# PaulTFLi/Machine-Learning-Replications

Hardware: AMD Instinct MI355X
Metric: train_rows_per_sec (higher is better)
Workload: dtype fp32

## Files before the change

machine-learning-replications_amd/ops/csrc/svm_ws.hip:

```cpp
#include <type_traits>

#include "common.h"

namespace hfens {

struct WsProb {
  long long zoff;
  long long aoff;
  int l;
  int npos;
  double Cp, Cn;
  float ngl2e;
  int pad;
};

struct WsState {
  int done;
  int outer;
  long long inner;
  double gap;
  int nc;
  int nws;
  int nprev;
  int pad;
// ... 86 lines not shown
  }
  *total = tot;
  return base;
}

__device__ __forceinline__ void hist_add(int* hist, bool on, int bin) {
  const unsigned long long act = __ballot(on);
  if (!act) return;
  const int first = __builtin_amdgcn_readlane(bin, __builtin_ctzll(act));
  const unsigned long long same = __ballot(on && bin == first);
  if (same == act) {
    if ((threadIdx.x & 63) == __builtin_ctzll(act)) atomicAdd(&hist[first], __popcll(act));
  } else if (on) {
    atomicAdd(&hist[bin], 1);
  }
}

struct WsAux {
  unsigned* keys;
  long long n;
  unsigned long long* gkey;
};

__device__ __forceinline__ unsigned ws_key(double v) { return f32_okey((float)v); }

__device__ __forceinline__ void ws_publish_keys(const WsProb& P, int b, int t, bool valid, double a, double g,
                                                const WsAux& X) {
  double su = -kWsInf, sl = -kWsInf;
  if (valid) {
    unsigned ku = 0u, kl = 0u;
    const bool pos = t < P.npos;
    const double C = pos ? P.Cp : P.Cn;
    const double yg = pos ? g : -g;
    if (pos ? a < C : a > 0) { su = -yg; ku = ws_key(su); }
    if (pos ? a > 0 : a < C) { sl = yg; kl = ws_key(sl); }
    X.keys[P.aoff + t] = ku;
    X.keys[X.n + P.aoff + t] = kl;
  }
  su = wave_max_f64_exact(su);
  sl = wave_max_f64_exact(sl);
  if ((threadIdx.x & 63) == 0) {
    if (su > -kWsInf) atomicMax(&X.gkey[2 * b], f64_okey(su));
    if (sl > -kWsInf) atomicMax(&X.gkey[2 * b + 1], f64_okey(sl));
  }
}

__global__ __launch_bounds__(256) void ws_init_kernel(const WsProb* __restrict__ probs, const float* __restrict__ zcat,
                                                      int F, float* __restrict__ zn, double* __restrict__ alpha,
                                                      double* __restrict__ G, WsState* __restrict__ states,
                                                      WsAux X) {
  const int b = blockIdx.y;
  const WsProb P = probs[b];
  const int t = blockIdx.x * blockDim.x + threadIdx.x;
  if (blockIdx.x * blockDim.x >= P.l) return;
  if (blockIdx.x == 0 && threadIdx.x == 0) states[b] = WsState{0, 0, 0, 0.0, 0, 0, 0, 0, 0, 0, 0, 0, 0, 0};
  const bool valid = t < P.l;
  if (valid) {
    const float* z = zcat + (P.zoff + t) * F;
    float s = 0.f;
    for (int k = 0; k < F; ++k) s = fmaf(z[k], z[k], s);
    zn[P.aoff + t] = s;
    alpha[P.aoff + t] = 0.0;
    G[P.aoff + t] = -1.0;
  }
  ws_publish_keys(P, b, t, valid, 0.0, -1.0, X);
}

constexpr size_t ws_sel_lds_bytes(int Q) { return 32 * 4 + 4096 * 4 + 1024 * 4 + (size_t)Q * 4; }

template <int M, typename Emit>
__device__ __forceinline__ int ws_pick_lists(const unsigned (&ku)[M], const unsigned (&kl)[M], int t0, int k_up,
                                             int k_low, int* shi, int* binfo, int* hist, Emit emit) {
  const int tid = threadIdx.x;
  for (int i = tid; i < 4096; i += kWsThreads) hist[i] = 0;
  if (tid < 8) binfo[tid] = 0;
  __syncthreads();
#pragma unroll
  for (int m = 0; m < M; ++m) {
    hist_add(hist, ku[m] != 0u, (int)(ku[m] >> 21));
    hist_add(hist, kl[m] != 0u, 2048 + (int)(kl[m] >> 21));
  }
  __syncthreads();
  ws_find_bin(hist, k_up, k_low, shi, binfo);
  __syncthreads();
  const unsigned bu1 = binfo[0], bl1 = binfo[2];
  const int au1 = binfo[1], al1 = binfo[3];
  for (int i = tid; i < 4096; i += kWsThreads) hist[i] = 0;
  __syncthreads();
#pragma unroll
  for (int m = 0; m < M; ++m) {
    hist_add(hist, ku[m] != 0u && (ku[m] >> 21) == bu1, (int)((ku[m] >> 10) & 2047));
    hist_add(hist, kl[m] != 0u && (kl[m] >> 21) == bl1, 2048 + (int)((kl[m] >> 10) & 2047));
  }
  __syncthreads();
  ws_find_bin(hist, k_up - au1, k_low - al1, shi, binfo + 4);
  __syncthreads();
  const unsigned Tu = (bu1 << 11) | (unsigned)binfo[4], Tl = (bl1 << 11) | (unsigned)binfo[6];
  const int need_u = k_up - au1 - binfo[5], need_l = k_low - al1 - binfo[7];
  unsigned selm = 0u;
  int base = 0;
#pragma unroll
  for (int side = 0; side < 2; ++side) {
    const unsigned T = side ? Tl : Tu;
    const int need = side ? need_l : need_u;
    int wt = 0;
#pragma unroll
    for (int m = 0; m < M; ++m) {
      const unsigned k = side ? kl[m] : ku[m];
      wt += __popcll(__ballot(k && (k >> 10) == T && !((selm >> m) & 1u)));
    }
    int ttot;
    int trank = wave_base(wt, shi, &ttot);
    unsigned pick = 0u;
    int ws_cnt = 0;
#pragma unroll
    for (int m = 0; m < M; ++m) {
      const unsigned k = side ? kl[m] : ku[m];
      const bool cand = k && !((selm >> m) & 1u);
      const bool tie = cand && (k >> 10) == T;
      const unsigned long long tb = __ballot(tie);
      const bool take = cand && ((k >> 10) > T || (tie && trank + __popcll(tb & lanes_below()) < need));
      trank += __popcll(tb);
      if (take) pick |= 1u << m;
      ws_cnt += __popcll(__ballot(take));
    }
    int stot;
    int pos = base + wave_base(ws_cnt, shi, &stot);
#pragma unroll
    for (int m = 0; m < M; ++m) {
      const bool take = (pick >> m) & 1u;
      const unsigned long long tb = __ballot(take);
      if (take) emit(pos + __popcll(tb & lanes_below()), t0 + 64 * m);
      pos += __popcll(tb);
    }
    selm |= pick;
    base += stot;
  }
  return base;
}

struct WsCand {
  int* idx;
  unsigned* ku;
  unsigned* kl;
  int ncand;
};
constexpr int kWsCandM = 8;
constexpr int kWsCandBlk = kWsCandM * kWsThreads;

template <int M, int Q, bool kWriteIdx, bool kCand = false>
__device__ __forceinline__ int ws_select_body(const WsProb& P, int b, WsState* S, int* __restrict__ wsidx,
                                              int* __restrict__ wsprev, double eps, int max_outer, const WsAux& X,
                                              int* shi, int* binfo, int* hist, unsigned* bm, int* widx,
                                              const WsCand& C = WsCand{nullptr, nullptr, nullptr, 0}) {
  const int nprev = S->nprev;
  const int tid = threadIdx.x;
  const int lane = tid & 63, wave = tid >> 6;
  const int L = kCand ? C.ncand : P.l;
  const int t0 = wave * 64 * M + lane;
  const long long c0 = __builtin_amdgcn_s_memtime();
  const unsigned long long gku = X.gkey[2 * b], gkl = X.gkey[2 * b + 1];
  const double Gmax = gku ? f64_from_okey(gku) : -kWsInf;
  const double Gmax2 = gkl ? f64_from_okey(gkl) : -kWsInf;
  const double gap = Gmax + Gmax2;
  unsigned ku[M], kl[M];
  int nu = 0, nl = 0;
#pragma unroll
  for (int m = 0; m < M; ++m) {
    const int t = t0 + 64 * m;
    if (kCand) {
      ku[m] = t < L ? C.ku[(size_t)b * C.ncand + t] : 0u;
      kl[m] = t < L ? C.kl[(size_t)b * C.ncand + t] : 0u;
    } else {
      ku[m] = t < L ? __builtin_nontemporal_load(X.keys + P.aoff + t) : 0u;
      kl[m] = t < L ? __builtin_nontemporal_load(X.keys + X.n + P.aoff + t) : 0u;
    }
  }
#pragma unroll
  for (int m = 0; m < M; ++m) {
    nu += __popcll(__ballot(ku[m] != 0u));
    nl += __popcll(__ballot(kl[m] != 0u));
  }
  if (!kCand)
    for (int i = tid; i < 1024; i += kWsThreads) bm[i] = 0;
  int n_up;
  wave_base(nu | (nl << 16), shi, &n_up);
  const int n_low = n_up >> 16;
  n_up &= 0xFFFF;
  if (!(gap >= eps) || S->outer >= max_outer || n_up == 0 || n_low == 0) {
    if (tid == 0) { S->done = 1; S->gap = gap; S->nc = 0; S->nws = 0; }
    return -1;
  }
  if (tid == 0) { X.gkey[2 * b] = 0ull; X.gkey[2 * b + 1] = 0ull; }
  const int k_up = min(Q / 4, n_up), k_low = min(Q / 4, n_low);
  const long long c0a = __builtin_amdgcn_s_memtime();
  const int nnew = ws_pick_lists<M>(ku, kl, t0, k_up, k_low, shi, binfo, hist, [&](int i, int p) {
    if (kCand) {
      widx[i] = C.idx[(size_t)b * C.ncand + p];
    } else {
      widx[i] = p;
      atomicOr(&bm[p >> 5], 1u << (p & 31));
    }
  });
  const long long c0b = __builtin_amdgcn_s_memtime();
  const long long c0c = c0b;
  __syncthreads();
  const int pv = tid < nprev ? wsprev[(size_t)b * (Q / 2) + tid] : -1;
  bool again = false;
  if (pv >= 0) {
    if (kCand) {
      for (int w = 0; w < nnew; ++w) again |= widx[w] == pv;
    } else {
      again = (bm[pv >> 5] >> (pv & 31)) & 1u;
    }
  }
  const bool keep = pv >= 0 && !again;
  const unsigned long long kb = __ballot(keep);
  int ktot;
  const int kpos = nnew + wave_base(__popcll(kb), shi, &ktot) + __popcll(kb & lanes_below());
  if (keep) widx[kpos] = pv;
  __syncthreads();
  const int nws = nnew + ktot;
  for (int w = tid; w < nnew; w += kWsThreads) wsprev[(size_t)b * (Q / 2) + w] = widx[w];
  if (kWriteIdx)
    for (int w = tid; w < nws; w += kWsThreads) wsidx[(size_t)b * Q + w] = widx[w];
  const long long c1 = __builtin_amdgcn_s_memtime();
  if (tid == 0) {
    S->cyc_select += c1 - c0;
    S->cyc_p0 += c0a - c0;
    S->cyc_p1 += c0b - c0a;
    S->cyc_p2 += c0c - c0b;
    S->nws = nws;
    S->nprev = nnew;
    S->gap = gap;
  }
  return nws;
}

template <int Q>
__global__ __launch_bounds__(kWsThreads) void ws_cand_kernel(const WsProb* __restrict__ probs,
                                                             const WsState* __restrict__ states, WsAux X, WsCand C) {
  constexpr int M = kWsCandM;
  constexpr int per = Q / 2;
  const int b = blockIdx.y, blk = blockIdx.x;
  if (states[b].done) return;
  const WsProb P = probs[b];
  const int tid = threadIdx.x;
  const int lane = tid & 63, wave = tid >> 6;
  const int beg = blk * kWsCandBlk;
  int* out_idx = C.idx + (size_t)b * C.ncand + (size_t)blk * per;
  unsigned* out_ku = C.ku + (size_t)b * C.ncand + (size_t)blk * per;
  unsigned* out_kl = C.kl + (size_t)b * C.ncand + (size_t)blk * per;
  __shared__ int shi[16], binfo[16];
  __shared__ int hist[4096];
  __shared__ int pick[per];
  const int t0 = wave * 64 * M + lane;
  unsigned ku[M], kl[M];
  int nu = 0, nl = 0;
#pragma unroll
  for (int m = 0; m < M; ++m) {
    const int t = beg + t0 + 64 * m;
    ku[m] = t < P.l ? __builtin_nontemporal_load(X.keys + P.aoff + t) : 0u;
    kl[m] = t < P.l ? __builtin_nontemporal_load(X.keys + X.n + P.aoff + t) : 0u;
  }
#pragma unroll
  for (int m = 0; m < M; ++m) {
    nu += __popcll(__ballot(ku[m] != 0u));
    nl += __popcll(__ballot(kl[m] != 0u));
  }
  int n_up;
  wave_base(nu | (nl << 16), shi, &n_up);
  const int n_low = n_up >> 16;
  n_up &= 0xFFFF;
  const int np = (n_up == 0 && n_low == 0) ? 0
                 : ws_pick_lists<M>(ku, kl, t0, min(Q / 4, n_up), min(Q / 4, n_low), shi, binfo, hist,
                                    [&](int i, int p) { pick[i] = beg + p; });
  __syncthreads();
  if (tid < per) {
    const int t = tid < np ? pick[tid] : -1;
    out_idx[tid] = t;
    out_ku[tid] = t >= 0 ? X.keys[P.aoff + t] : 0u;
    out_kl[tid] = t >= 0 ? X.keys[X.n + P.aoff + t] : 0u;
  }
}

template <int M, int Q>
__global__ __launch_bounds__(kWsThreads) void ws_select_kernel(
    const WsProb* __restrict__ probs, WsState* __restrict__ states, int* __restrict__ wsidx,
    int* __restrict__ wsprev, double eps, int max_outer, WsAux X) {
  const int b = blockIdx.x;
  WsState* S = states + b;
  if (S->done) return;
  const WsProb P = probs[b];
  extern __shared__ __attribute__((aligned(16))) unsigned char ws_lds[];
  int* shi = reinterpret_cast<int*>(ws_lds);
  int* binfo = shi + 16;
  int* hist = shi + 32;
  unsigned* bm = reinterpret_cast<unsigned*>(hist + 4096);
  int* widx = reinterpret_cast<int*>(bm + 1024);
  ws_select_body<M, Q, true>(P, b, S, wsidx, wsprev, eps, max_outer, X, shi, binfo, hist, bm, widx);
}

constexpr size_t ws_solve_lds_bytes(int Q, int FP) {
  return 64 * 4 + (size_t)Q * FP * 4 + (size_t)Q * 4 * 2 + (size_t)6 * Q * 4;
}

template <int FP, int Q, int TH>
__global__ __launch_bounds__(TH) void ws_solve_kernel(
    const WsProb* __restrict__ probs, WsState* __restrict__ states, const float* __restrict__ zcat, int F,
    const float* __restrict__ zn_all, double* __restrict__ alpha_all, const double* __restrict__ G_all,
    const int* __restrict__ wsidx, float* __restrict__ wsz, float* __restrict__ wsn, float* __restrict__ wdc,
    int Fp2, double eps, int max_inner, double inner_frac, long long* __restrict__ prof) {
  static_assert(Q % TH == 0 && (Q & (Q - 1)) == 0 && TH % 64 == 0 && TH <= 512, "whole slots per thread");
  static_assert(FP % 4 == 0, "z rows are read as float4");
  constexpr int SL = Q / TH;
  static_assert(SL % 2 == 0, "slots go in pairs (packed f32 fma)");
  constexpr int NW = TH / 64;
  constexpr unsigned kIdx = Q - 1;
  const int b = blockIdx.x;
  WsState* S = states + b;
  if (S->done) return;
  const WsProb P = probs[b];
  const int nws = S->nws;
  const int tid = threadIdx.x;
  const int lane = tid & 63, wave = tid >> 6;
  extern __shared__ __attribute__((aligned(16))) unsigned char ws_lds[];
  unsigned* red = reinterpret_cast<unsigned*>(ws_lds);
  float* zB = reinterpret_cast<float*>(ws_lds + 64 * 4);
  float* snB = zB + (size_t)Q * FP;
  int* widx = reinterpret_cast<int*>(snB + Q);
  float* gl = reinterpret_cast<float*>(widx + Q);
  float* al = gl + 2 * Q;
  float* kil = al + 2 * Q;
  const double* Gp = G_all + P.aoff;
  double* ap = alpha_all + P.aoff;
  const long long c1 = __builtin_amdgcn_s_memtime();
  {
    int wi[SL];
#pragma unroll
    for (int m = 0; m < SL; ++m) {
      const int s = tid + TH * m;
      wi[m] = s < nws ? wsidx[(size_t)b * Q + s] : -1;
    }
    float zv[SL][FP];
    float znv[SL];
#pragma unroll
    for (int m = 0; m < SL; ++m) {
      const float* zrow = zcat + (P.zoff + (wi[m] < 0 ? 0 : wi[m])) * F;
#pragma unroll
      for (int k = 0; k < FP; ++k) zv[m][k] = (wi[m] >= 0 && k < F) ? zrow[k] : 0.f;
      znv[m] = wi[m] >= 0 ? zn_all[P.aoff + wi[m]] : 0.f;
    }
#pragma unroll
    for (int m = 0; m < SL; ++m) {
      const int s = tid + TH * m;
      widx[s] = wi[m] < 0 ? 0 : wi[m];
      snB[s] = P.ngl2e * znv[m];
#pragma unroll
      for (int k = 0; k < FP; k += 4)
        *reinterpret_cast<f32x4*>(&zB[s * FP + k]) = f32x4{zv[m][k], zv[m][k + 1], zv[m][k + 2], zv[m][k + 3]};
    }
  }
  __syncthreads();
  const long long c2 = __builtin_amdgcn_s_memtime();
  const long long r2 = __builtin_amdgcn_s_memrealtime();
  bool valid[SL], pos[SL];
  int tt[SL];
  float y[SL], Cw[SL], a[SL], yg[SL], sn[SL], tu[SL], tl[SL];
  double a0[SL];
  f32x2 zp[SL / 2][FP];
#pragma unroll
  for (int m = 0; m < SL; ++m) {
    const int s = tid + TH * m;
    valid[m] = s < nws;
    tt[m] = valid[m] ? widx[s] : 0;
    pos[m] = tt[m] < P.npos;
    y[m] = pos[m] ? 1.f : -1.f;
    Cw[m] = (float)(pos[m] ? P.Cp : P.Cn);
    tu[m] = valid[m] ? (pos[m] ? Cw[m] : 0.f) : -INFINITY;
    tl[m] = valid[m] ? (pos[m] ? 0.f : Cw[m]) : -INFINITY;
    a0[m] = valid[m] ? ap[tt[m]] : 0.0;
    a[m] = (float)a0[m];
    yg[m] = valid[m] ? y[m] * (float)Gp[tt[m]] : 0.f;
    sn[m] = valid[m] ? snB[s] : 0.f;
#pragma unroll
    for (int k = 0; k < FP; k += 4) {
      const f32x4 v = valid[m] ? *reinterpret_cast<const f32x4*>(&zB[s * FP + k]) : f32x4{0.f, 0.f, 0.f, 0.f};
#pragma unroll
      for (int q = 0; q < 4; ++q) zp[m / 2][k + q][m & 1] = v[q];
    }
  }
  const float k2c = -2.f * P.ngl2e;
  const float Cpf = (float)P.Cp, Cnf = (float)P.Cn;
  auto krow = [&](int r, float (&out)[SL]) {
    f32x2 d[SL / 2];
#pragma unroll
    for (int h = 0; h < SL / 2; ++h) d[h] = f32x2{0.f, 0.f};
#pragma unroll
    for (int k = 0; k < FP; k += 4) {
      const f32x4 v = *reinterpret_cast<const f32x4*>(&zB[r * FP + k]);
#pragma unroll
      for (int q = 0; q < 4; ++q) {
#pragma unroll
        for (int h = 0; h < SL / 2; ++h) d[h] = __builtin_elementwise_fma(f32x2{v[q], v[q]}, zp[h][k + q], d[h]);
      }
    }
    const float snr = snB[r];
#pragma unroll
    for (int m = 0; m < SL; ++m)
      out[m] = __builtin_amdgcn_exp2f(fminf(fmaf(k2c, d[m / 2][m & 1], snr + sn[m]), 0.f));
  };
  auto red4 = [&](const unsigned* r) {
    unsigned x = 0u;
#pragma unroll
    for (int w = 0; w < NW; w += 4) {
      const uint4 v = *reinterpret_cast<const uint4*>(r + w);
      x = max(max(x, max(v.x, v.y)), max(v.z, v.w));
    }
    return x;
  };
  float tol_in = -1.f;
  const float epsf = (float)eps;
#ifdef HFENS_WS_STAMPS
  const bool pf = prof != nullptr;
  long long ph[6] = {0, 0, 0, 0, 0, 0};
  long long tp = pf ? __builtin_amdgcn_s_memtime() : 0;
#define WS_STAMP(k)                                         \
  if (pf) {                                                 \
    const long long tn = __builtin_amdgcn_s_memtime();      \
    ph[k] += tn - tp;                                       \
    tp = tn;                                                \
  }
#else
  const bool pf = false;
  long long ph[6] = {0, 0, 0, 0, 0, 0};
#define WS_STAMP(k)
#endif
  int it = 0;
  auto pair = [&](auto parc) -> bool {
    constexpr int par = decltype(parc)::value;
    float* glp = gl + par * Q;
    float* alp = al + par * Q;
    float* kip = kil + par * Q;
    unsigned* r1 = red + (0 * 2 + par) * NW;
    unsigned* r3 = red + (1 * 2 + par) * NW;
    unsigned* r2 = red + (2 * 2 + par) * NW;
    unsigned* r4 = red + (3 * 2 + par) * NW;
    unsigned k1 = 0u, k3 = 0u, k4 = 0u;
    bool low[SL];
#pragma unroll
    for (int m = 0; m < SL; ++m) {
      const unsigned s = (unsigned)(tid + TH * m);
      glp[s] = yg[m];
      alp[s] = a[m];
      const float ya = y[m] * a[m];
      const bool up = ya < tu[m];
      low[m] = -ya < tl[m];
      const unsigned um = 0u - (unsigned)up, lm = 0u - (unsigned)low[m];
      const unsigned kv = f32_okey(-yg[m]) & um;
      k4 = max(k4, kv);
      k1 = max(k1, ((kv & ~kIdx) | s) & um);
      k3 = max(k3, f32_okey(yg[m]) & lm);
    }
    k1 = wave_max_u32(k1);
    k3 = wave_max_u32(k3);
    k4 = wave_max_u32(k4);
    if (lane == 0) { r1[wave] = k1; r3[wave] = k3; r4[wave] = k4; }
    WS_STAMP(0)
    __syncthreads();
    const unsigned K1 = __builtin_amdgcn_readfirstlane(red4(r1));
    const unsigned K3 = __builtin_amdgcn_readfirstlane(red4(r3));
    const unsigned K4 = __builtin_amdgcn_readfirstlane(red4(r4));
    if (K1 == 0u || K3 == 0u) return false;
    const int i = (int)(K1 & kIdx);
    const float ygi = glp[i];
    const bool ipos = widx[i] < P.npos;
    const float yi = ipos ? 1.f : -1.f;
    const float Gi = yi * ygi;
    const float GmaxB = -ygi;
    const float lgap = f32_from_okey(K4) + f32_from_okey(K3);
    if (tol_in < 0.f) tol_in = fmaxf(0.9999f * epsf, (float)inner_frac * lgap);
    if (lgap < tol_in) return false;
    WS_STAMP(1)
    float Ki[SL];
    krow(i, Ki);
    unsigned k2 = 0u;
#pragma unroll
    for (int m = 0; m < SL; ++m) {
      const unsigned s = (unsigned)(tid + TH * m);
      kip[s] = Ki[m];
      const float gd = GmaxB + yg[m];
      const float q0 = 2.f - 2.f * Ki[m];
      const float quad = q0 <= 0.f ? 1e-12f : q0;
      const unsigned ok = 0u - (unsigned)(low[m] & (gd > 0.f));
      k2 = max(k2, ((f32_okey(gd * gd * __builtin_amdgcn_rcpf(quad)) & ~kIdx) | s) & ok);
    }
    k2 = wave_max_u32(k2);
    if (lane == 0) r2[wave] = k2;
    WS_STAMP(2)
    __syncthreads();
    const unsigned K2 = __builtin_amdgcn_readfirstlane(red4(r2));
    if (K2 == 0u) return false;
    const int j = (int)(K2 & kIdx);
    const float ai_old = alp[i], aj_old = alp[j];
    const float Kij = kip[j];
    const bool jpos = widx[j] < P.npos;
    const float yj = jpos ? 1.f : -1.f;
    const float Gj = yj * glp[j];
    const float Ci = ipos ? Cpf : Cnf, Cj = jpos ? Cpf : Cnf;
    WS_STAMP(3)
    const float q0 = 2.f - 2.f * Kij;
    const float rq = __builtin_amdgcn_rcpf(q0 <= 0.f ? 1e-12f : q0);
    float ao, bo, as, bs;
    {
      const float delta = (-Gi - Gj) * rq;
      const float diff = ai_old - aj_old;
      ao = ai_old + delta;
      bo = aj_old + delta;
      const bool c1 = (diff > 0.f) & (bo < 0.f), c2 = !(diff > 0.f) & (ao < 0.f);
      ao = c1 ? diff : (c2 ? 0.f : ao);
      bo = c1 ? 0.f : (c2 ? -diff : bo);
      const bool c3 = (diff > Ci - Cj) & (ao > Ci), c4 = !(diff > Ci - Cj) & (bo > Cj);
      ao = c3 ? Ci : (c4 ? Cj + diff : ao);
      bo = c3 ? Ci - diff : (c4 ? Cj : bo);
    }
    {
      const float delta = (Gi - Gj) * rq;
      const float sum = ai_old + aj_old;
      as = ai_old - delta;
      bs = aj_old + delta;
      const bool c1 = (sum > Ci) & (as > Ci), c2 = !(sum > Ci) & (bs < 0.f);
      as = c1 ? Ci : (c2 ? sum : as);
      bs = c1 ? sum - Ci : (c2 ? 0.f : bs);
      const bool c3 = (sum > Cj) & (bs > Cj), c4 = !(sum > Cj) & (as < 0.f);
      as = c3 ? sum - Cj : (c4 ? 0.f : as);
      bs = c3 ? Cj : (c4 ? sum : bs);
    }
    const bool opp = ipos != jpos;
    const float ai = opp ? ao : as, aj = opp ? bo : bs;
    const float ci = yi * (ai - ai_old), cj = yj * (aj - aj_old);
    WS_STAMP(4)
    float Kj[SL];
    krow(j, Kj);
#pragma unroll
    for (int m = 0; m < SL; ++m) {
      const int s = tid + TH * m;
      a[m] = s == i ? ai : (s == j ? aj : a[m]);
      yg[m] += fmaf(Ki[m], ci, Kj[m] * cj);
    }
    WS_STAMP(5)
    ++it;
    return true;
  };
  while (it < max_inner && pair(std::integral_constant<int, 0>{}) && it < max_inner &&
         pair(std::integral_constant<int, 1>{})) {
  }
#undef WS_STAMP
  if (pf && tid == 0) {
#pragma unroll
    for (int k = 0; k < 6; ++k) prof[(size_t)b * 6 + k] += ph[k];
  }
  int nc = 0;
#pragma unroll
  for (int m = 0; m < SL; ++m) {
    const int s = tid + TH * m;
    double anew = a0[m];
    if (valid[m] && a[m] != (float)a0[m]) {
      const double C = pos[m] ? P.Cp : P.Cn;
      anew = a[m] <= 0.f ? 0.0 : (a[m] >= Cw[m] ? C : a0[m] + ((double)a[m] - (double)(float)a0[m]));
    }
    const bool ch = valid[m] && anew != a0[m];
    const unsigned long long cm = __ballot(ch);
    __syncthreads();
    if (lane == 0) red[wave] = (unsigned)__popcll(cm);
    __syncthreads();
    int wb = 0, tot = 0;
#pragma unroll
    for (int w = 0; w < NW; ++w) {
      const int v = (int)red[w];
      wb += w < wave ? v : 0;
      tot += v;
    }
    const int cpos = nc + wb + __popcll(cm & lanes_below());
    if (ch) {
      ap[tt[m]] = anew;
      for (int k = 0; k < Fp2; ++k) wsz[((size_t)b * Fp2 + k) * Q + cpos] = k < F ? zB[s * FP + k] : 0.f;
      wsn[(size_t)b * Q + cpos] = sn[m];
      wdc[(size_t)b * Q + cpos] = (float)((double)y[m] * (anew - a0[m]));
    }
    nc += tot;
  }
  const int ncp = (nc + 31) & ~31;
  for (int p = nc + tid; p < ncp; p += TH) {
    for (int k = 0; k < Fp2; ++k) wsz[((size_t)b * Fp2 + k) * Q + p] = 0.f;
    wsn[(size_t)b * Q + p] = 0.f;
    wdc[(size_t)b * Q + p] = 0.f;
  }
  const long long c3 = __builtin_amdgcn_s_memtime();
  const long long r3 = __builtin_amdgcn_s_memrealtime();
  if (tid == 0) {
    S->cyc_build += c2 - c1;
    S->cyc_inner += c3 - c2;
    S->cyc_p2 += r3 - r2;
    if (it == 0 || nc == 0) S->done = 1;
    S->nc = nc;
    S->outer += 1;
    S->inner += it;
  }
}

__device__ __forceinline__ unsigned sel4u(const unsigned (&v)[4], int m) {
  const unsigned m0 = 0u - (unsigned)(m == 0), m1 = 0u - (unsigned)(m == 1);
  const unsigned m2 = 0u - (unsigned)(m == 2), m3 = 0u - (unsigned)(m == 3);
  return (v[0] & m0) | (v[1] & m1) | (v[2] & m2) | (v[3] & m3);
}

constexpr int kKcQ = 256;
constexpr int kKcQP = kKcQ + 1;
constexpr int kKcTri = kKcQ * (kKcQ + 1) / 2;
constexpr size_t kc_zbuf_bytes(int KS) {
  return (size_t)2 * KS * kKcQP * 4 > (4096 + 1024) * 4 ? (size_t)2 * KS * kKcQP * 4 : (4096 + 1024) * 4;
}
constexpr size_t kc_lds_bytes(int KS) { return 128 + 2 * kKcQ * 4 + (kc_zbuf_bytes(KS) + 15) / 16 * 16 + (size_t)kKcTri * 4; }
static_assert(kc_lds_bytes(12) <= 163840, "the K-cached round must fit the CU's 160 KiB of LDS");

__device__ __forceinline__ int kc_rowstart(int r) { return r * kKcQ - ((r * (r - 1)) >> 1); }

__device__ __forceinline__ float sel4(const float (&v)[4], int m) {
  const unsigned u[4] = {__float_as_uint(v[0]), __float_as_uint(v[1]), __float_as_uint(v[2]), __float_as_uint(v[3])};
  return __uint_as_float(sel4u(u, m));
}
__device__ __forceinline__ int sel4(const int (&v)[4], int m) {
  const unsigned u[4] = {(unsigned)v[0], (unsigned)v[1], (unsigned)v[2], (unsigned)v[3]};
  return (int)sel4u(u, m);
}
__device__ __forceinline__ float rdlane_f(float v, int l) { return __int_as_float(__builtin_amdgcn_readlane(__float_as_int(v), l)); }

template <int M, int KS, bool kCand, bool kStamp = false>
__global__ __launch_bounds__(kWsThreads) void ws_kc_round_kernel(
    const WsProb* __restrict__ probs, WsState* __restrict__ states, const float* __restrict__ zcat, int F,
    const float* __restrict__ zn_all, double* __restrict__ alpha_all, const double* __restrict__ G_all,
    int* __restrict__ wsprev, float* __restrict__ wsz, float* __restrict__ wsn, float* __restrict__ wdc,
    int Fp2, double eps, int max_outer, int max_inner, double inner_frac, WsAux X, WsCand C,
    long long* __restrict__ prof = nullptr) {
  constexpr int Q = kKcQ;
  constexpr int SL = Q / 64;
  constexpr unsigned kIdx = Q - 1;
  static_assert(SL == 4, "sel4 assumes four slots per lane");
  const int b = blockIdx.x;
  WsState* S = states + b;
  if (S->done) return;
  const WsProb P = probs[b];
  const int tid = threadIdx.x;
  const int lane = tid & 63, wave = tid >> 6;
  extern __shared__ __attribute__((aligned(16))) unsigned char ws_lds[];
  int* shi = reinterpret_cast<int*>(ws_lds);
  int* binfo = shi + 16;
  int* widx = shi + 32;
  float* snB = reinterpret_cast<float*>(widx + Q);
  float* zbuf = snB + Q;
  int* hist = reinterpret_cast<int*>(zbuf);
  unsigned* bm = reinterpret_cast<unsigned*>(hist + 4096);
  float* tri = zbuf + (kc_zbuf_bytes(KS) + 15) / 16 * 4;
  const int nws = ws_select_body<M, Q, false, kCand>(P, b, S, nullptr, wsprev, eps, max_outer, X, shi, binfo,
                                                     hist, bm, widx, C);
  if (nws < 0) return;
  const long long c1 = __builtin_amdgcn_s_memtime();
  for (int e = tid; e < 2 * KS * Q; e += kWsThreads) {
    const int k = e / Q, s = e - k * Q;
    zbuf[k * kKcQP + s] = (s < nws && k < F) ? zcat[(P.zoff + widx[s]) * F + k] : 0.f;
  }
  if (tid < Q) snB[tid] = tid < nws ? P.ngl2e * zn_all[P.aoff + widx[tid]] : 0.f;
  __syncthreads();
  {
    const int r32 = lane & 31, hi = lane >> 5;
    const float k2 = -2.f * P.ngl2e;
    for (int t = wave; t < 36; t += kWsWaves) {
      int ta = 0, rem = t;
      while (rem >= 8 - ta) { rem -= 8 - ta; ++ta; }
      const int tb = ta + rem;
      f32x16 A = {0.f};
#pragma unroll
      for (int q = 0; q < KS; ++q) {
        const float* zr = zbuf + (2 * q + hi) * kKcQP;
        A = __builtin_amdgcn_mfma_f32_32x32x2f32(zr[ta * 32 + r32], zr[tb * 32 + r32], A, 0, 0, 0);
      }
      const int col = tb * 32 + r32;
      const float snc = snB[col];
#pragma unroll
      for (int r = 0; r < 16; ++r) {
        const int row = ta * 32 + 8 * (r >> 2) + 4 * hi + (r & 3);
        const float kv = __builtin_amdgcn_exp2f(fminf(fmaf(k2, A[r], snB[row] + snc), 0.f));
        if (row <= col) tri[kc_rowstart(row) + col - row] = kv;
      }
    }
  }
  __syncthreads();
  const long long c2 = __builtin_amdgcn_s_memtime();
  if (wave != 0) return;
  const double* Gp = G_all + P.aoff;
  double* ap = alpha_all + P.aoff;
  bool valid[SL], pos[SL];
  int tt[SL], rb[SL];
  float y[SL], Cw[SL], a[SL], yg[SL], tu[SL], tl[SL];
  double a0[SL];
#pragma unroll
  for (int m = 0; m < SL; ++m) {
    const int s = 64 * m + lane;
    valid[m] = s < nws;
    tt[m] = valid[m] ? widx[s] : 0;
    pos[m] = tt[m] < P.npos;
    y[m] = pos[m] ? 1.f : -1.f;
    Cw[m] = (float)(pos[m] ? P.Cp : P.Cn);
    tu[m] = valid[m] ? (pos[m] ? Cw[m] : 0.f) : -INFINITY;
    tl[m] = valid[m] ? (pos[m] ? 0.f : Cw[m]) : -INFINITY;
    a0[m] = valid[m] ? ap[tt[m]] : 0.0;
    a[m] = (float)a0[m];
    yg[m] = valid[m] ? y[m] * (float)Gp[tt[m]] : 0.f;
    rb[m] = kc_rowstart(s) - s;
  }
  auto krow = [&](int r, float (&out)[SL]) {
    const int ra = kc_rowstart(r) - r;
#pragma unroll
    for (int m = 0; m < SL; ++m) {
      const int s = 64 * m + lane;
      out[m] = tri[s >= r ? ra + s : rb[m] + r];
    }
  };
  const float Cpf = (float)P.Cp, Cnf = (float)P.Cn;
  const float epsf = (float)eps;
  float tol_in = -1.f;
  int it = 0;
  long long ph[5] = {0, 0, 0, 0, 0};
  long long tp = kStamp ? (long long)__builtin_amdgcn_s_memtime() : 0;
  auto stamp = [&](int k) {
    if constexpr (kStamp) {
      const long long tn = __builtin_amdgcn_s_memtime();
      ph[k] += tn - tp;
      tp = tn;
    }
  };
  while (it < max_inner) {
    unsigned k1 = 0u, k3 = 0u;
    bool low[SL];
#pragma unroll
    for (int m = 0; m < SL; ++m) {
      const unsigned s = (unsigned)(64 * m + lane);
      const float ya = y[m] * a[m];
      const bool up = ya < tu[m];
      low[m] = -ya < tl[m];
      const unsigned um = 0u - (unsigned)up, lm = 0u - (unsigned)low[m];
      k1 = max(k1, ((f32_okey(-yg[m]) & ~kIdx) | s) & um);
      k3 = max(k3, f32_okey(yg[m]) & lm);
    }
    const unsigned K1 = __builtin_amdgcn_readfirstlane(wave_max_u32(k1));
    const unsigned K3 = __builtin_amdgcn_readfirstlane(wave_max_u32(k3));
    stamp(0);
    if (K1 == 0u || K3 == 0u) break;
    const int i = (int)(K1 & kIdx), mi = i >> 6, li = i & 63;
    const float ygi = rdlane_f(sel4(yg, mi), li);
    const float ai_old = rdlane_f(sel4(a, mi), li);
    const bool ipos = __builtin_amdgcn_readlane(sel4(tt, mi), li) < P.npos;
    const float yi = ipos ? 1.f : -1.f;
    const float Gi = yi * ygi;
    const float GmaxB = -ygi;
    const float lgap = GmaxB + f32_from_okey(K3);
    if (tol_in < 0.f) tol_in = fmaxf(0.9999f * epsf, (float)inner_frac * lgap);
    if (lgap < tol_in) break;
    float Ki[SL];
    krow(i, Ki);
    stamp(1);
    unsigned k2 = 0u;
#pragma unroll
    for (int m = 0; m < SL; ++m) {
      const unsigned s = (unsigned)(64 * m + lane);
      const float gd = GmaxB + yg[m];
      const float q0 = 2.f - 2.f * Ki[m];
      const float quad = q0 <= 0.f ? 1e-12f : q0;
      const unsigned ok = 0u - (unsigned)(low[m] & (gd > 0.f));
      k2 = max(k2, ((f32_okey(gd * gd * __builtin_amdgcn_rcpf(quad)) & ~kIdx) | s) & ok);
    }
    const unsigned K2 = __builtin_amdgcn_readfirstlane(wave_max_u32(k2));
    stamp(2);
    if (K2 == 0u) break;
    const int j = (int)(K2 & kIdx), mj = j >> 6, lj = j & 63;
    float Kj[SL];
    krow(j, Kj);
    const float ygj = rdlane_f(sel4(yg, mj), lj);
    const float aj_old = rdlane_f(sel4(a, mj), lj);
    const float Kij = rdlane_f(sel4(Ki, mj), lj);
    const bool jpos = __builtin_amdgcn_readlane(sel4(tt, mj), lj) < P.npos;
    const float yj = jpos ? 1.f : -1.f;
    const float Gj = yj * ygj;
    const float Ci = ipos ? Cpf : Cnf, Cj = jpos ? Cpf : Cnf;
    const float q0 = 2.f - 2.f * Kij;
    const float rq = __builtin_amdgcn_rcpf(q0 <= 0.f ? 1e-12f : q0);
    float ao, bo, as, bs;
    {
      const float delta = (-Gi - Gj) * rq;
      const float diff = ai_old - aj_old;
      ao = ai_old + delta;
      bo = aj_old + delta;
      const bool c1 = (diff > 0.f) & (bo < 0.f), c2 = !(diff > 0.f) & (ao < 0.f);
      ao = c1 ? diff : (c2 ? 0.f : ao);
      bo = c1 ? 0.f : (c2 ? -diff : bo);
      const bool c3 = (diff > Ci - Cj) & (ao > Ci), c4 = !(diff > Ci - Cj) & (bo > Cj);
      ao = c3 ? Ci : (c4 ? Cj + diff : ao);
      bo = c3 ? Ci - diff : (c4 ? Cj : bo);
    }
    {
      const float delta = (Gi - Gj) * rq;
      const float sum = ai_old + aj_old;
      as = ai_old - delta;
      bs = aj_old + delta;
      const bool c1 = (sum > Ci) & (as > Ci), c2 = !(sum > Ci) & (bs < 0.f);
      as = c1 ? Ci : (c2 ? sum : as);
      bs = c1 ? sum - Ci : (c2 ? 0.f : bs);
      const bool c3 = (sum > Cj) & (bs > Cj), c4 = !(sum > Cj) & (as < 0.f);
      as = c3 ? sum - Cj : (c4 ? 0.f : as);
      bs = c3 ? Cj : (c4 ? sum : bs);
    }
    const bool opp = ipos != jpos;
    const float ai = opp ? ao : as, aj = opp ? bo : bs;
    const float ci = yi * (ai - ai_old), cj = yj * (aj - aj_old);
    stamp(3);
#pragma unroll
    for (int m = 0; m < SL; ++m) {
      const int s = 64 * m + lane;
      a[m] = s == i ? ai : (s == j ? aj : a[m]);
      yg[m] += fmaf(Ki[m], ci, Kj[m] * cj);
    }
    stamp(4);
    ++it;
  }
  if constexpr (kStamp) {
    if (lane == 0)
      for (int k = 0; k < 5; ++k) prof[(size_t)b * 6 + k] += ph[k];
  }
  int nc = 0;
#pragma unroll
  for (int m = 0; m < SL; ++m) {
    const int s = 64 * m + lane;
    double anew = a0[m];
    if (valid[m] && a[m] != (float)a0[m]) {
      const double C = pos[m] ? P.Cp : P.Cn;
      anew = a[m] <= 0.f ? 0.0 : (a[m] >= Cw[m] ? C : a0[m] + ((double)a[m] - (double)(float)a0[m]));
// ... 503 lines not shown
```

Baseline: 622,200.

## Restructure WS solve LDS mirrors into slot-contiguous vector stores and hoist row loads

Per-slot mirrors of yg, alpha and kernel row now go into a thread-contiguous LDS layout written with a single vector store per thread, and y and sn are cached there too, so scalar loads for i and j come from one base address. The z-row and scalars for the selected i and j are loaded right after the first reduction, ahead of the remaining reductions and the early-exit checks, which are deferred into a combined stop flag. This aims to cut LDS store instructions and hide LDS latency on the serial critical path of each SMO pair step. In exchange the kernel uses more LDS and holds extra registers for the z-row, and the stop decision now comes after the second reduction, so one extra krow and barrier run on the final iteration.

```diff
diff --git a/machine-learning-replications_amd/ops/csrc/svm_ws.hip b/machine-learning-replications_amd/ops/csrc/svm_ws.hip
--- a/machine-learning-replications_amd/ops/csrc/svm_ws.hip
+++ b/machine-learning-replications_amd/ops/csrc/svm_ws.hip
@@ -412,7 +412,16 @@
 }
 
 constexpr size_t ws_solve_lds_bytes(int Q, int FP) {
-  return 64 * 4 + (size_t)Q * FP * 4 + (size_t)Q * 4 * 2 + (size_t)6 * Q * 4;
+  return 64 * 4 + (size_t)Q * FP * 4 + (size_t)Q * 4 * 2 + (size_t)8 * Q * 4;
+}
+
+template <int SL>
+__device__ __forceinline__ void ws_store_slots(float* p, const float (&v)[SL]) {
+  typedef float vec __attribute__((ext_vector_type(SL)));
+  vec x;
+#pragma unroll
+  for (int m = 0; m < SL; ++m) x[m] = v[m];
+  *reinterpret_cast<vec*>(p) = x;
 }
 
 template <int FP, int Q, int TH>
@@ -439,9 +448,8 @@
   float* zB = reinterpret_cast<float*>(ws_lds + 64 * 4);
   float* snB = zB + (size_t)Q * FP;
   int* widx = reinterpret_cast<int*>(snB + Q);
-  float* gl = reinterpret_cast<float*>(widx + Q);
-  float* al = gl + 2 * Q;
-  float* kil = al + 2 * Q;
+  float* ysn = reinterpret_cast<float*>(widx + Q);
+  float* mir = ysn + 2 * Q;
   const double* Gp = G_all + P.aoff;
   double* ap = alpha_all + P.aoff;
   const long long c1 = __builtin_amdgcn_s_memtime();
@@ -500,22 +508,23 @@
       for (int q = 0; q < 4; ++q) zp[m / 2][k + q][m & 1] = v[q];
     }
   }
+  ws_store_slots<SL>(ysn + tid * SL, y);
+  ws_store_slots<SL>(ysn + Q + tid * SL, sn);
   const float k2c = -2.f * P.ngl2e;
   const float Cpf = (float)P.Cp, Cnf = (float)P.Cn;
-  auto krow = [&](int r, float (&out)[SL]) {
+  auto krow = [&](const f32x4 (&zr)[FP / 4], float snr, float (&out)[SL]) {
     f32x2 d[SL / 2];
 #pragma unroll
     for (int h = 0; h < SL / 2; ++h) d[h] = f32x2{0.f, 0.f};
 #pragma unroll
     for (int k = 0; k < FP; k += 4) {
-      const f32x4 v = *reinterpret_cast<const f32x4*>(&zB[r * FP + k]);
+      const f32x4 v = zr[k / 4];
 #pragma unroll
       for (int q = 0; q < 4; ++q) {
 #pragma unroll
         for (int h = 0; h < SL / 2; ++h) d[h] = __builtin_elementwise_fma(f32x2{v[q], v[q]}, zp[h][k + q], d[h]);
       }
     }
-    const float snr = snB[r];
 #pragma unroll
     for (int m = 0; m < SL; ++m)
       out[m] = __builtin_amdgcn_exp2f(fminf(fmaf(k2c, d[m / 2][m & 1], snr + sn[m]), 0.f));
@@ -549,28 +558,28 @@
   int it = 0;
   auto pair = [&](auto parc) -> bool {
     constexpr int par = decltype(parc)::value;
-    float* glp = gl + par * Q;
-    float* alp = al + par * Q;
-    float* kip = kil + par * Q;
+    float* mp = mir + par * 3 * Q;
+    constexpr int oG = (2 + 3 * par) * Q, oA = oG + Q, oK = oA + Q;
     unsigned* r1 = red + (0 * 2 + par) * NW;
     unsigned* r3 = red + (1 * 2 + par) * NW;
     unsigned* r2 = red + (2 * 2 + par) * NW;
     unsigned* r4 = red + (3 * 2 + par) * NW;
     unsigned k1 = 0u, k3 = 0u, k4 = 0u;
     bool low[SL];
+    ws_store_slots<SL>(mp + tid * SL, yg);
+    ws_store_slots<SL>(mp + Q + tid * SL, a);
 #pragma unroll
     for (int m = 0; m < SL; ++m) {
       const unsigned s = (unsigned)(tid + TH * m);
-      glp[s] = yg[m];
-      alp[s] = a[m];
       const float ya = y[m] * a[m];
       const bool up = ya < tu[m];
       low[m] = -ya < tl[m];
       const unsigned um = 0u - (unsigned)up, lm = 0u - (unsigned)low[m];
-      const unsigned kv = f32_okey(-yg[m]) & um;
+      const unsigned ky = f32_okey(yg[m]);
+      const unsigned kv = ~ky & um;
       k4 = max(k4, kv);
       k1 = max(k1, ((kv & ~kIdx) | s) & um);
-      k3 = max(k3, f32_okey(yg[m]) & lm);
+      k3 = max(k3, ky & lm);
     }
     k1 = wave_max_u32(k1);
     k3 = wave_max_u32(k3);
@@ -579,26 +588,30 @@
     WS_STAMP(0)
     __syncthreads();
     const unsigned K1 = __builtin_amdgcn_readfirstlane(red4(r1));
+    const int i = (int)(K1 & kIdx);
+    const int ti = (i & (TH - 1)) * SL + i / TH;
+    const float* bi = ysn + ti;
+    const float sni = bi[Q], ygi = bi[oG], ai_old = bi[oA], yi = bi[0];
+    f32x4 zi[FP / 4];
+#pragma unroll
+    for (int k = 0; k < FP; k += 4) zi[k / 4] = *reinterpret_cast<const f32x4*>(&zB[i * FP + k]);
+    __builtin_amdgcn_sched_barrier(0);
     const unsigned K3 = __builtin_amdgcn_readfirstlane(red4(r3));
     const unsigned K4 = __builtin_amdgcn_readfirstlane(red4(r4));
-    if (K1 == 0u || K3 == 0u) return false;
-    const int i = (int)(K1 & kIdx);
-    const float ygi = glp[i];
-    const bool ipos = widx[i] < P.npos;
-    const float yi = ipos ? 1.f : -1.f;
+    const bool ipos = yi > 0.f;
     const float Gi = yi * ygi;
     const float GmaxB = -ygi;
     const float lgap = f32_from_okey(K4) + f32_from_okey(K3);
     if (tol_in < 0.f) tol_in = fmaxf(0.9999f * epsf, (float)inner_frac * lgap);
-    if (lgap < tol_in) return false;
+    const bool stop = (K1 == 0u) | (K3 == 0u) | (lgap < tol_in);
     WS_STAMP(1)
     float Ki[SL];
-    krow(i, Ki);
+    krow(zi, sni, Ki);
+    ws_store_slots<SL>(mp + 2 * Q + tid * SL, Ki);
     unsigned k2 = 0u;
 #pragma unroll
     for (int m = 0; m < SL; ++m) {
       const unsigned s = (unsigned)(tid + TH * m);
-      kip[s] = Ki[m];
       const float gd = GmaxB + yg[m];
       const float q0 = 2.f - 2.f * Ki[m];
       const float quad = q0 <= 0.f ? 1e-12f : q0;
@@ -610,13 +623,17 @@
     WS_STAMP(2)
     __syncthreads();
     const unsigned K2 = __builtin_amdgcn_readfirstlane(red4(r2));
-    if (K2 == 0u) return false;
+    if (stop || K2 == 0u) return false;
     const int j = (int)(K2 & kIdx);
-    const float ai_old = alp[i], aj_old = alp[j];
-    const float Kij = kip[j];
-    const bool jpos = widx[j] < P.npos;
-    const float yj = jpos ? 1.f : -1.f;
-    const float Gj = yj * glp[j];
+    const int tj = (j & (TH - 1)) * SL + j / TH;
+    const float* bj = ysn + tj;
+    const float Kij = bj[oK], ygj = bj[oG], aj_old = bj[oA], yj = bj[0], snj = bj[Q];
+    f32x4 zj[FP / 4];
+#pragma unroll
+    for (int k = 0; k < FP; k += 4) zj[k / 4] = *reinterpret_cast<const f32x4*>(&zB[j * FP + k]);
+    __builtin_amdgcn_sched_barrier(0);
+    const bool jpos = yj > 0.f;
+    const float Gj = yj * ygj;
     const float Ci = ipos ? Cpf : Cnf, Cj = jpos ? Cpf : Cnf;
     WS_STAMP(3)
     const float q0 = 2.f - 2.f * Kij;
@@ -651,7 +668,7 @@
     const float ci = yi * (ai - ai_old), cj = yj * (aj - aj_old);
     WS_STAMP(4)
     float Kj[SL];
-    krow(j, Kj);
+    krow(zj, snj, Kj);
 #pragma unroll
     for (int m = 0; m < SL; ++m) {
       const int s = tid + TH * m;
```

Result: faster. 638,900 (median of 6 runs) (+2.7%).
